# google/lasr

Hardware: AMD Instinct MI355X
Metric: rasterizer fwd+bwd frames/sec at 256x256, 2.3k faces (higher is better)
Workload: dtype f32

## Files before the change

lasr_amd/csrc/sr_backward.h:

```cpp
#pragma once
#include "sr_common.h"

namespace lasr {

constexpr bool BWD_FM = true;
#ifndef LASR_BWD_LDSREC
#define LASR_BWD_LDSREC 1
#endif
#ifndef LASR_BWD_WPE8
#define LASR_BWD_WPE8 0
#endif
#ifndef LASR_BWD_DIVREC
#define LASR_BWD_DIVREC 1
#endif
#ifndef LASR_BWD_ONE
#define LASR_BWD_ONE 1
#endif
constexpr int QCAP = 128;
constexpr int BWD_THREADS = 64;

template <bool LASR_FAST, int NCH>
__global__ __launch_bounds__(BWD_THREADS)
#if LASR_BWD_WPE8
__attribute__((amdgpu_waves_per_eu(LASR_FAST && NCH == 3 ? 8 : 1, LASR_FAST && NCH == 3 ? 8 : 8)))
#endif
void sr_backward_kernel(RasterArgs A, const float* __restrict__ colors,
                                                          const float* __restrict__ aggrs,
                                                          const float* __restrict__ gcolors,
                                                          float* __restrict__ gfaces, float* __restrict__ gtex)
{
    __shared__ unsigned int s_ring[BWD_THREADS / 64][QCAP];
#if LASR_BWD_LDSREC
    __shared__ __attribute__((aligned(16))) float s_rec[BWD_THREADS / 64][REC];
#endif
    constexpr bool FM = BWD_FM;
    const Modes m = LASR_FAST ? Modes{2, 1, 2, 1, 1} : A.m;
    if (A.near_far_dev) { A.near = A.near_far_dev[0]; A.far = A.near_far_dev[1]; }
    const int lane = threadIdx.x & 63;
    unsigned int* ring = s_ring[threadIdx.x >> 6];
#if defined(LASR_BWD_ORDER) && LASR_BWD_ORDER == 1
    int blk = xcd_remap(blockIdx.x, gridDim.x);
    {
        const int total = gridDim.x, per = total >> 3;
        if ((total & 7) == 0 && per % A.F == 0) {
            const int m = per / A.F, i = blockIdx.x >> 3, rank = i / m;
            blk = ((blockIdx.x & 7) * m + (i - rank * m)) * A.F + rank;
        }
    }
#elif defined(LASR_BWD_ORDER) && LASR_BWD_ORDER == 3
    const int blk = xcd_remap(blockIdx.x, gridDim.x);
#else
    int blk;
    {
        const int total = gridDim.x, per = total >> 3;
        blk = (total & 7) == 0 ? (blockIdx.x & 7) * per + (per - 1 - (blockIdx.x >> 3)) : total - 1 - blockIdx.x;
    }
#endif
    const int gw = __builtin_amdgcn_readfirstlane((int)((blk * blockDim.x + threadIdx.x) >> 6));
    if (gw >= A.N * A.F) return;
    const int bn = gw / A.F, fn = gw - bn * A.F;
    const int IS = A.IS, P = IS * IS;
    const cptr_t rec = as_const(A.recs + (size_t)gw * REC);
    const cptr_t tex = as_const(A.textures + (size_t)gw * A.T * NCH);
    const int flags = __float_as_int(rec[R_FLAGS]);
#if LASR_BWD_LDSREC
    typedef const float __attribute__((address_space(3)))* lptr_t;
    if (LASR_FAST && (flags & 16)) {
        float* dst = s_rec[threadIdx.x >> 6];
        if (lane < REC) dst[lane] = A.recs[(size_t)gw * REC + lane];
        __builtin_amdgcn_wave_barrier();
    }
    const lptr_t lrec = (lptr_t)s_rec[threadIdx.x >> 6];
#endif

    const unsigned rlo = (unsigned)__float_as_int(rec[R_BB + 0]), rext = (unsigned)__float_as_int(rec[R_BB + 1]);
    const int x0 = (int)(rlo & 0xffff), r0 = (int)(rlo >> 16);
    const int bw = (int)(rext & 0xffff) + 1, bh = (int)(rext >> 16) + 1;
    const bool empty = rlo == 0xffffffffu;
    const int npx = empty ? 0 : bw * bh;

    float gv[9] = {0, 0, 0, 0, 0, 0, 0, 0, 0};
    constexpr int NGT = 3 * NCH < 18 ? 18 : 3 * NCH;
    constexpr int THIRD = NCH == 9 ? 18 : 0;
    float gt[NGT];
#pragma unroll
    for (int k = 0; k < NGT; k++) gt[k] = 0.f;
    const bool front = (flags & 8) != 0;
    const bool vertex_tex = (m.tex == 1);
    const int lim = (A.N * A.F - gw) * A.T;
    const bool use_far = (m.dist == 2) && (flags & 16);
    const float thr_pad = A.thr * 1.05f;
    const float inv_is = A.inv_is;
    const bool pow2 = (IS & (IS - 1)) == 0;
    const float cx_a = A.cx_a, cx_b = A.cx_b, cy_b = A.cy_b;
    auto centre_x = [&](int xi) { return OPT_BWD_S1 && pow2 ? __builtin_fmaf((float)xi, cx_a, cx_b) : pix_center_p2(xi, IS, inv_is, pow2); };
    auto centre_y = [&](int row) { return OPT_BWD_S1 && pow2 ? __builtin_fmaf((float)row, -cx_a, cy_b) : pix_center_p2(IS - 1 - row, IS, inv_is, pow2); };
    float ld[9];
    const float far_t = A.far_t;
    if (OPT_BWD_S1 && use_far) {
#pragma unroll
        for (int k = 0; k < 3; k++) {
            const float h = __builtin_amdgcn_sqrtf(rec[R_HK2 + k]);
            ld[3 * k] = rec[R_INV + 3 * k] * h; ld[3 * k + 1] = rec[R_INV + 3 * k + 1] * h; ld[3 * k + 2] = rec[R_INV + 3 * k + 2] * h;
        }
    }
    const float tie_scale = (flags & 16) ? near_tie_scale(rec[R_HK2], rec[R_HK2 + 1], rec[R_HK2 + 2]) : 0.f;
    bool depth_safe = false;
    if (OPT_BWD_MATH && (flags & 16)) {
        const float z0 = rec[R_FACE + 2], z1 = rec[R_FACE + 5], z2 = rec[R_FACE + 8];
        const float zlo = fminf(fminf(z0, z1), z2), zhi = fmaxf(fmaxf(z0, z1), z2);
        depth_safe = zlo > 0.f && zlo * (1.f - 1e-4f) > A.near && zhi * (1.f + 1e-4f) < A.far;
    }
    auto ld_plane = [&](const float* base, int nplanes, int plane, int pn_) -> float {
#if defined(LASR_BWD_ABL) && LASR_BWD_ABL == 3
        return 0.25f + 1e-3f * (float)(pn_ & 255) + 0.01f * (float)plane;
#endif
        return base[((size_t)bn * nplanes + plane) * P + pn_];
    };

    int r = 0, c = 0;
#if LASR_BWD_DIVREC
    const int walk = __float_as_int(rec[15]);
    const int dr = empty ? 0 : walk >> 17, dc = empty ? 0 : 64 - dr * bw;
    if (!empty) { r = (lane * (walk & 0x1ffff)) >> 16; c = lane - r * bw; }
#else
    const int dr = empty ? 0 : 64 / bw, dc = empty ? 0 : 64 - dr * bw;
    if (!empty) { r = lane / bw; c = lane - r * bw; }
#endif

    int head = 0, tail = 0, base = 0;
    while (true) {
        if (base < npx) {
            const int xi = x0 + c, row = r0 + r;
            const bool in_range = base + lane < npx;
            c += dc; r += dr;
            if (c >= bw) { c -= bw; r += 1; }
            base += 64;
            bool keep = in_range;
            if (OPT_BWD_S1) {
                if (use_far) {
                    const float xp = __builtin_fmaf((float)xi, cx_a, cx_b), yp = __builtin_fmaf((float)row, -cx_a, cy_b);
                    const float d0 = __builtin_fmaf(ld[0], xp, __builtin_fmaf(ld[1], yp, ld[2]));
                    const float d1 = __builtin_fmaf(ld[3], xp, __builtin_fmaf(ld[4], yp, ld[5]));
                    const float d2 = __builtin_fmaf(ld[6], xp, __builtin_fmaf(ld[7], yp, ld[8]));
                    keep = in_range && !(fminf(fminf(d0, d1), d2) < far_t);
                }
            } else if (in_range && use_far) {
                float w0, w1, w2;
                barycentric(rec, pix_center_p2(xi, IS, inv_is, pow2), pix_center_p2(IS - 1 - row, IS, inv_is, pow2), w0, w1, w2);
                keep = !certainly_far(rec, w0, w1, w2, thr_pad);
            }
            const unsigned long long mask = wave_mask(keep);
            if (keep) ring[(tail + bits_below_lane(mask)) & (QCAP - 1)] = (unsigned)xi | ((unsigned)row << 16);
            tail += __popcll(mask);
        }
        const int avail = tail - head;
        if (!(avail >= 64 || (base >= npx && avail > 0))) {
            if (base >= npx) break;
            continue;
        }
        __builtin_amdgcn_wave_barrier();
        const bool active = lane < avail;
        const unsigned int packed = ring[(head + lane) & (QCAP - 1)];
        head += min(avail, 64);
#if defined(LASR_BWD_ABL) && LASR_BWD_ABL == 1
        gv[0] += (float)packed;
        continue;
#endif
        if (!active) continue;
        const int xi = packed & 0xffff, row = packed >> 16;
        const int pn = row * IS + xi;
        const float xp = centre_x(xi), yp = centre_y(row);

        float w0, w1, w2;
        Frag fr;
#if LASR_BWD_ONE
        if (LASR_FAST && (flags & 16)) {
#if LASR_BWD_LDSREC
            if (!fragment_one(lrec, A.thr, A.sigma, xp, yp, w0, w1, w2, fr, tie_scale)) continue;
#else
            if (!fragment_one(rec, A.thr, A.sigma, xp, yp, w0, w1, w2, fr, tie_scale)) continue;
#endif
        } else
#endif
        if (!fragment<FM, cptr_t, (OPT_BWD_MATH && LASR_FAST)>(rec, m.dist, A.thr, A.sigma, xp, yp, w0, w1, w2, fr)) continue;
        const float D = fr.D;
#if defined(LASR_BWD_ABL) && LASR_BWD_ABL == 2
        gv[0] += D + fr.dx + fr.dy + fr.t0 + fr.t1 + fr.t2 + fr.sign;
        continue;
#endif

        float Ca = ld_plane(gcolors, NCH + 1, NCH, pn);
        if (m.alpha == 1) Ca = div_<FM>(Ca, (float)A.F);
        else if (m.alpha == 2) {
            const float a_out = ld_plane(colors, NCH + 1, NCH, pn);
            Ca *= div_<FM>(1 - a_out, fmaxf(1 - D, 1e-6f));
        }
        float C = Ca;

        const float u0 = w0, u1 = w1, u2 = w2;
        if (vertex_tex) clip_normalise<FM, (OPT_BWD_MATH && LASR_FAST)>(w0, w1, w2); else clip_normalise<false>(w0, w1, w2);
        const float iz0r = rec[R_IZ + 0], iz1r = rec[R_IZ + 1], iz2r = rec[R_IZ + 2];
        const float q0 = w0 * iz0r, q1 = w1 * iz1r, q2 = w2 * iz2r;
        const float zp = OPT_BWD_MATH && LASR_FAST ? __builtin_amdgcn_rcpf(q0 + q1 + q2) : depth_at<FM>(rec, w0, w1, w2);
        if (!depth_safe) {
            float zc = zp;
            const float tol = 1e-4f * fabsf(zp);
            if (fabsf(zp - A.near) <= tol || fabsf(zp - A.far) <= tol) zc = depth_forward_exact(rec, xp, yp);
            if (zc < A.near || zc > A.far) continue;
        }

        float gz0 = 0, gz1 = 0, gz2 = 0;
        if (m.rgb == 0) {
            if ((float)fn == ld_plane(aggrs, 2, 1, pn)) {
                float g[NCH];
#pragma unroll
                for (int k = 0; k < NCH; k++) g[k] = ld_plane(gcolors, NCH + 1, k, pn);
                if (vertex_tex) {
#pragma unroll
                    for (int k = 0; k < NCH; k++) {
                        gt[k] += w0 * g[k]; gt[NCH + k] += w1 * g[k]; gt[2 * NCH + k] += w2 * g[k];
                    }
                } else {
                    const int j = surface_texel(w0, w1, A.res);
                    if (j >= 0 && j < A.T) {
                        float* gtp = gtex + (size_t)gw * A.T * 3 + 3 * j;
                        atomicAdd(gtp + 0, g[0]); atomicAdd(gtp + 1, g[1]); atomicAdd(gtp + 2, g[2]);
                    }
                }
            }
        } else if (front || m.double_side) {
            const float ssum = ld_plane(aggrs, 2, 0, pn);
            const float smax = ld_plane(aggrs, 2, 1, pn);
            const float zn = div_<FM>(A.far - zp, A.far - A.near);
            const float sm = div_<FM>(D * exp_<FM>(div_<FM>(zn - smax, A.gamma)), ssum);
            float g[NCH];
#pragma unroll
            for (int k = 0; k < NCH; k++) g[k] = ld_plane(gcolors, NCH + 1, k, pn);
            if (vertex_tex) {
#pragma unroll
                for (int k = 0; k < NCH; k++) {
                    gt[k] += sm * (w0 * g[k]); gt[NCH + k] += sm * (w1 * g[k]); gt[2 * NCH + k] += sm * (w2 * g[k]);
                }
            } else {
                const int j = surface_texel(w0, w1, A.res);
                if (j >= 0 && j < A.T) {
                    float* gtp = gtex + (size_t)gw * A.T * 3 + 3 * j;
                    atomicAdd(gtp + 0, sm * g[0]); atomicAdd(gtp + 1, sm * g[1]); atomicAdd(gtp + 2, sm * g[2]);
                }
            }
            float Crgb = 0.f;
#pragma unroll
            for (int k = 0; k < NCH; k++)
                Crgb += g[k] * (sample_colour(tex, w0, w1, w2, A.res, k, m.tex, lim, NCH) - ld_plane(colors, NCH + 1, k, pn));
            Crgb *= sm;
            C += div_<FM>(Crgb, D);
            const float Cz = div_<FM>(div_<FM>(Crgb, A.gamma), A.near - A.far) * zp * zp;
            if (OPT_BWD_MATH && LASR_FAST) {
                gz0 = Cz * q0 * iz0r; gz1 = Cz * q1 * iz1r; gz2 = Cz * q2 * iz2r;
            } else {
                const float iz0 = __builtin_amdgcn_rcpf(rec[R_FACE + 2]), iz1 = __builtin_amdgcn_rcpf(rec[R_FACE + 5]), iz2 = __builtin_amdgcn_rcpf(rec[R_FACE + 8]);
                gz0 = Cz * w0 * iz0 * iz0;
                gz1 = Cz * w1 * iz1 * iz1;
                gz2 = Cz * w2 * iz2 * iz2;
            }
        }

        C *= div_<FM>(D * (1 - D), A.sigma);
        float gx0 = 0, gy0 = 0, gx1 = 0, gy1 = 0, gx2 = 0, gy2 = 0;
        if (m.dist == 1) {
            const float t0 = fr.t0, t1 = fr.t1, t2 = fr.t2;
            const int p = t0 > t1 ? (t1 > t2 ? 2 : 1) : (t0 > t2 ? 2 : 0);
            const float ipx = rec[R_INV + 3 * p + 0], ipy = rec[R_INV + 3 * p + 1];
            const float dis = fr.dis;
            const float sc = 2.f * sqrtf(fabsf(dis));
            float gxy[3][2];
#pragma unroll
            for (int l = 0; l < 2; l++) {
                const float ipl = l == 0 ? ipx : ipy;
#pragma unroll
                for (int k = 0; k < 3; k++) {
                    float acc = 0.f;
                    acc += -ipl * rec[R_INV + 3 * k + 0] * xp;
                    acc += -ipl * rec[R_INV + 3 * k + 1] * yp;
                    acc += -ipl * rec[R_INV + 3 * k + 2] * 1.f;
                    gxy[k][l] = acc * C * sc;
                }
            }
            gx0 = gxy[0][0]; gy0 = gxy[0][1]; gx1 = gxy[1][0]; gy1 = gxy[1][1]; gx2 = gxy[2][0]; gy2 = gxy[2][1];
        } else if (m.dist == 2) {
            const float k2 = 2 * fr.sign * C;
            gx0 = k2 * (fr.t0 + u0) * fr.dx; gy0 = k2 * (fr.t0 + u0) * fr.dy;
            gx1 = k2 * (fr.t1 + u1) * fr.dx; gy1 = k2 * (fr.t1 + u1) * fr.dy;
            gx2 = k2 * (fr.t2 + u2) * fr.dx; gy2 = k2 * (fr.t2 + u2) * fr.dy;
        }
        gv[0] += gx0; gv[1] += gy0; gv[2] += gz0;
        gv[3] += gx1; gv[4] += gy1; gv[5] += gz1;
        gv[6] += gx2; gv[7] += gy2; gv[8] += gz2;
    }

    float v18[18], red[5];
    const int lane_row = lane >> 4;
    const int sub = lane_row == 0 ? 0 : lane_row == 1 ? 2 : lane_row == 2 ? 1 : 3;
    float* gf = gfaces + (size_t)gw * 9;
    float* gtp = gtex + (size_t)gw * 3 * NCH;
#pragma unroll
    for (int pass = 0; pass < (NCH > 3 ? 2 : 1); pass++) {
#pragma unroll
        for (int k = 0; k < 9; k++) {
            v18[k] = pass == 0 ? gv[k] : (vertex_tex ? gt[9 + k] : 0.f);
            v18[9 + k] = pass == 0 ? (vertex_tex ? gt[k] : 0.f) : (NCH == 9 && vertex_tex ? gt[THIRD + k] : 0.f);
        }
        wave_reduce18(v18, red);
        if ((lane & 15) == 15) {
#pragma unroll
            for (int i = 0; i < 5; i++) {
                if (i == 4 && (lane_row & 1)) continue;
                const int comp = i == 4 ? 16 + (lane_row >> 1) : 4 * i + sub;
                const bool ow = A.overwrite_grads && vertex_tex;
                if (pass == 0) {
                    if (comp < 9) gf[comp] = ow ? red[i] : gf[comp] + red[i];
                    else if (vertex_tex) gtp[comp - 9] = ow ? red[i] : gtp[comp - 9] + red[i];
                } else if ((comp < 9 || NCH == 9) && vertex_tex) gtp[9 + comp] = ow ? red[i] : gtp[9 + comp] + red[i];
            }
        }
    }
}

}
```

lasr_amd/csrc/sr_device.h:

```cpp
#pragma once
#include <hip/hip_runtime.h>

namespace lasr {

constexpr int REC = 48;

#ifndef LASR_OPT
#define LASR_OPT 0xffff
#endif
constexpr bool OPT_PKRECT = (LASR_OPT & 1) != 0;
constexpr bool OPT_MED3 = (LASR_OPT & 2) != 0;
constexpr bool OPT_NOSCALE = (LASR_OPT & 4) != 0;
constexpr bool OPT_SIGNFOLD = (LASR_OPT & 8) != 0;
constexpr bool OPT_SOFTMAX = (LASR_OPT & 16) != 0;
constexpr bool OPT_BWD_S1 = (LASR_OPT & 64) != 0;
constexpr bool OPT_BWD_MATH = (LASR_OPT & 128) != 0;
constexpr bool OPT_EDGESEL = (LASR_OPT & 256) != 0;
constexpr int R_BB = 0, R_FLAGS = 2, R_INV = 3, R_HK2 = 12, R_FACE = 16, R_DEN = 25, R_IDEN = 28, R_E = 32, R_IZ = 41;

typedef const float __attribute__((address_space(4)))* cptr_t;
__device__ __forceinline__ cptr_t as_const(const float* p) { return (cptr_t)(unsigned long long)p; }

struct Modes {
    int dist, rgb, alpha, tex, double_side;
// ... 189 lines not shown
    y = __builtin_fmaf(__builtin_fmaf(-b, y, 1.f), y, y);
#define LASR_QUOT(a)                                                     \
    {                                                                    \
        float q = a * y;                                                 \
        q = __builtin_fmaf(__builtin_fmaf(-b, q, a), y, q);              \
        a = __builtin_fmaf(__builtin_fmaf(-b, q, a), y, q);              \
    }
    LASR_QUOT(a0) LASR_QUOT(a1) LASR_QUOT(a2)
#undef LASR_QUOT
}

template <bool FM = false, bool TAME = false>
__device__ __forceinline__ void clip_normalise(float& w0, float& w1, float& w2)
{
    if (TAME) {
        w0 = __builtin_amdgcn_fmed3f(w0, 0.f, 1.f);
        w1 = __builtin_amdgcn_fmed3f(w1, 0.f, 1.f);
        w2 = __builtin_amdgcn_fmed3f(w2, 0.f, 1.f);
    } else {
        w0 = fmaxf(fminf(w0, 1.f), 0.f);
        w1 = fmaxf(fminf(w1, 1.f), 0.f);
        w2 = fmaxf(fminf(w2, 1.f), 0.f);
    }
    const float s = fmaxf(w0 + w1 + w2, 1e-5f);
    if (FM) { const float r = __builtin_amdgcn_rcpf(s); w0 *= r; w1 *= r; w2 *= r; }
    else div3_shared(w0, w1, w2, s);
}

template <bool FM> __device__ __forceinline__ float div_(float a, float b)
{
    return FM ? a * __builtin_amdgcn_rcpf(b) : a / b;
}
__device__ __forceinline__ float exp_1ulp(float x)
{
    const float L2E_HI = 1.44269502162933349609375f, L2E_LO = 1.925963033500011e-8f;
    const float n = rintf(x * L2E_HI);
    const float f = __builtin_fmaf(x, L2E_LO, __builtin_fmaf(x, L2E_HI, -n));
    return ldexpf(__builtin_amdgcn_exp2f(f), (int)n);
}
template <bool FM> __device__ __forceinline__ float exp_(float x) { return FM ? __expf(x) : exp_1ulp(x); }
template <bool FM, bool NOSCALE = false> __device__ __forceinline__ float sigmoid_neg_(float neg_arg)
{
    if (FM) return __builtin_amdgcn_rcpf(1.f + __expf(neg_arg));
    if (NOSCALE) return (float)recip64_noscale(1. + (double)exp_1ulp(neg_arg));
    return (float)(1. / (1. + (double)exp_1ulp(neg_arg)));
}

template <typename RP>
__device__ __forceinline__ bool certainly_far(RP rec, float w0, float w1, float w2, float thr_pad)
{
    return (w0 < 0.f && w0 * w0 * rec[R_HK2 + 0] > thr_pad) ||
           (w1 < 0.f && w1 * w1 * rec[R_HK2 + 1] > thr_pad) ||
           (w2 < 0.f && w2 * w2 * rec[R_HK2 + 2] > thr_pad);
}

template <int K, bool CLAMP, bool FM = false, bool MK = false, typename RP = cptr_t, bool IDEN = false>
__device__ __forceinline__ void edge_project(RP rec, float w0, float w1, float w2,
                                             float& u0, float& u1, float& u2)
{
#pragma clang fp contract(off)
    constexpr int B = (K + 1) % 3;
    const float e0 = rec[R_E + 3 * K + 0], e1 = rec[R_E + 3 * K + 1], e2 = rec[R_E + 3 * K + 2];
    const float eb = rec[R_E + 3 * K + B];
    const float num = w0 * e0 + w1 * e1 + w2 * e2 - eb;
    float ta = MK ? div_by_recip(num, rec[R_DEN + K], rec[R_IDEN + K])
                  : (FM && IDEN) ? num * rec[R_IDEN + K] : div_<FM>(num, rec[R_DEN + K]);
    float tb = 1 - ta;
    float tc = 0;
    if (CLAMP) {
        ta = fminf(fmaxf(ta, 0.f), 1.f);
        tb = fminf(fmaxf(tb, 0.f), 1.f);
    }
    float t[3];
    t[K] = ta; t[B] = tb; t[(K + 2) % 3] = tc;
    u0 = t[0] - w0; u1 = t[1] - w1; u2 = t[2] - w2;
}

struct Frag {
    float D;
    float sign, dx, dy;
    float t0, t1, t2;
    float dis;
    float narg;
};

template <bool FM = false, bool MK = false, typename RP = cptr_t, bool FWD = false, bool TAME = false, bool IDEN = false>
__device__ __forceinline__ bool euclid(RP rec, float xp, float yp,
                                       float w0, float w1, float w2, Frag& fr, float thr = 0.f)
{
#pragma clang fp contract(off)
    const float x0 = rec[R_FACE + 0], y0 = rec[R_FACE + 1], x1 = rec[R_FACE + 3], y1 = rec[R_FACE + 4], x2 = rec[R_FACE + 6], y2 = rec[R_FACE + 7];
    const bool inside = TAME ? (bool)((int)(fminf(fminf(w0, w1), w2) > 0) & (int)(fmaxf(fmaxf(w0, w1), w2) < 1))
                             : (w0 > 0 && w1 > 0 && w2 > 0 && w0 < 1 && w1 < 1 && w2 < 1);
    if (inside) {
        float best = 100000000.f, bx = 0, by = 0, b0 = 0, b1 = 0, b2 = 0;
        float u0, u1, u2;
#define LASR_TRY_EDGE(K)                                                          \
        edge_project<K, false, FM, MK, RP, IDEN>(rec, w0, w1, w2, u0, u1, u2);            \
        {                                                                         \
            const float px = u0 * x0 + u1 * x1 + u2 * x2;                         \
            const float py = u0 * y0 + u1 * y1 + u2 * y2;                         \
            const float d2 = px * px + py * py;                                   \
            if (d2 < best) { best = d2; bx = px; by = py; b0 = u0; b1 = u1; b2 = u2; } \
        }
        LASR_TRY_EDGE(0) LASR_TRY_EDGE(1) LASR_TRY_EDGE(2)
#undef LASR_TRY_EDGE
        if (FWD) { fr.narg = (-bx) * bx - by * by; return true; }
        fr.dx = bx; fr.dy = by; fr.t0 = b0; fr.t1 = b1; fr.t2 = b2; fr.sign = 1.f;
    } else {
        const int flags = __float_as_int(rec[R_FLAGS]);
        float u0, u1, u2;
        if (OPT_EDGESEL) {
            const bool n0 = w0 <= 0, n1 = w1 <= 0, n2 = w2 <= 0;
            bool o0 = false, o1 = false, o2 = false;
            if (flags & 7) {
                if (flags & 1) o0 = (xp - x0) * (x2 - x0) + (yp - y0) * (y2 - y0) > 0;
                if (flags & 2) o1 = (xp - x1) * (x0 - x1) + (yp - y1) * (y0 - y1) > 0;
                if (flags & 4) o2 = (xp - x2) * (x1 - x2) + (yp - y2) * (y1 - y2) > 0;
            }
            const bool c12 = n1 & n2, c20 = n2 & n0 & !n1, c01 = n0 & n1 & !n2;
            const bool e1 = (c20 & !o1) | (c01 & o2) | (n0 & !n1 & !n2);
            const bool e2 = (c01 & !o2) | (c12 & o0) | (n1 & !n0 & !n2);
            const bool e0 = !(e1 | e2);
            if (e0) edge_project<0, true, FM, MK, RP, IDEN>(rec, w0, w1, w2, u0, u1, u2);
            if (e1) edge_project<1, true, FM, MK, RP, IDEN>(rec, w0, w1, w2, u0, u1, u2);
            if (e2) edge_project<2, true, FM, MK, RP, IDEN>(rec, w0, w1, w2, u0, u1, u2);
        } else {
        int a = -1;
        if (w1 <= 0 && w2 <= 0) {
            a = 0;
            if ((flags & 1) && (xp - x0) * (x2 - x0) + (yp - y0) * (y2 - y0) > 0) a = 2;
        } else if (w2 <= 0 && w0 <= 0) {
            a = 1;
            if ((flags & 2) && (xp - x1) * (x0 - x1) + (yp - y1) * (y0 - y1) > 0) a = 0;
        } else if (w0 <= 0 && w1 <= 0) {
            a = 2;
            if ((flags & 4) && (xp - x2) * (x1 - x2) + (yp - y2) * (y1 - y2) > 0) a = 1;
        } else if (w0 <= 0) a = 1;
        else if (w1 <= 0) a = 2;
        else if (w2 <= 0) a = 0;
        if (a < 0) a = 0;
        if (a == 0) edge_project<0, true, FM, MK, RP, IDEN>(rec, w0, w1, w2, u0, u1, u2);
        else if (a == 1) edge_project<1, true, FM, MK, RP, IDEN>(rec, w0, w1, w2, u0, u1, u2);
        else edge_project<2, true, FM, MK, RP, IDEN>(rec, w0, w1, w2, u0, u1, u2);
        }
        fr.dx = u0 * x0 + u1 * x1 + u2 * x2;
        fr.dy = u0 * y0 + u1 * y1 + u2 * y2;
        if (FWD) { fr.narg = fr.dx * fr.dx + fr.dy * fr.dy; return !(fr.narg >= thr); }
        fr.t0 = u0; fr.t1 = u1; fr.t2 = u2; fr.sign = -1.f;
    }
    return true;
}

constexpr float NEAR_TIE = 0.985f;
constexpr float NEAR_TIE_ABS = 2.4e-6f;
__host__ __device__ __forceinline__ float near_tie_scale(float h2a, float h2b, float h2c)
{
    return 4.f * NEAR_TIE_ABS * NEAR_TIE_ABS / fminf(fminf(h2a, h2b), h2c);
}
__device__ __forceinline__ bool near_tie(float qlo, float qmid, float scale)
{
    const float gap = qmid - qlo;
    return (bool)((int)!(qlo < NEAR_TIE * qmid) | (int)!(gap * gap > scale * qmid));
}
#ifndef LASR_BWD_FMA
#define LASR_BWD_FMA 0
#endif
template <int K, typename RP>
__device__ __forceinline__ void edge_project_one(RP rec, float w0, float w1, float w2, float& u0, float& u1, float& u2)
{
#if !LASR_BWD_FMA
#pragma clang fp contract(off)
#endif
    constexpr int B = (K + 1) % 3;
    const float num = w0 * rec[R_E + 3 * K + 0] + w1 * rec[R_E + 3 * K + 1] + w2 * rec[R_E + 3 * K + 2] - rec[R_E + 3 * K + B];
    float ta = num * rec[R_IDEN + K];
    float tb = 1 - ta;
    ta = fminf(fmaxf(ta, 0.f), 1.f);
    tb = fminf(fmaxf(tb, 0.f), 1.f);
    float t[3];
    t[K] = ta; t[B] = tb; t[(K + 2) % 3] = 0;
    u0 = t[0] - w0; u1 = t[1] - w1; u2 = t[2] - w2;
}
template <typename RP>
__device__ __forceinline__ void euclid_one(RP rec, float xp, float yp, float w0, float w1, float w2, Frag& fr, float tie_scale)
{
#if !LASR_BWD_FMA
#pragma clang fp contract(off)
#endif
    const float x0 = rec[R_FACE + 0], y0 = rec[R_FACE + 1], x1 = rec[R_FACE + 3], y1 = rec[R_FACE + 4], x2 = rec[R_FACE + 6], y2 = rec[R_FACE + 7];
    const bool inside = (bool)((int)(fminf(fminf(w0, w1), w2) > 0) & (int)(fmaxf(fmaxf(w0, w1), w2) < 1));
    const int flags = __float_as_int(rec[R_FLAGS]);
    const bool n0 = w0 <= 0, n1 = w1 <= 0, n2 = w2 <= 0;
    bool o0 = false, o1 = false, o2 = false;
    if (flags & 7) {
        if (flags & 1) o0 = (xp - x0) * (x2 - x0) + (yp - y0) * (y2 - y0) > 0;
        if (flags & 2) o1 = (xp - x1) * (x0 - x1) + (yp - y1) * (y0 - y1) > 0;
        if (flags & 4) o2 = (xp - x2) * (x1 - x2) + (yp - y2) * (y1 - y2) > 0;
    }
    const bool c12 = n1 & n2, c20 = n2 & n0 & !n1, c01 = n0 & n1 & !n2;
    bool e1 = (c20 & !o1) | (c01 & o2) | (n0 & !n1 & !n2);
    bool e2 = (c01 & !o2) | (c12 & o0) | (n1 & !n0 & !n2);
    const float q0 = w2 * w2 * rec[R_HK2 + 2], q1 = w0 * w0 * rec[R_HK2 + 0], q2 = w1 * w1 * rec[R_HK2 + 1];
    const float qlo = fminf(fminf(q0, q1), q2), qmid = __builtin_amdgcn_fmed3f(q0, q1, q2);
    const bool tie = (bool)((int)inside & (int)near_tie(qlo, qmid, tie_scale));
    float u0, u1, u2;
    if (tie) {
        float best = 100000000.f, bx = 0, by = 0, b0 = 0, b1 = 0, b2 = 0;
#define LASR_TRY_EDGE(K)                                                          \
        edge_project<K, false, true, false, RP, true>(rec, w0, w1, w2, u0, u1, u2);   \
        {                                                                         \
            const float px = u0 * x0 + u1 * x1 + u2 * x2;                         \
            const float py = u0 * y0 + u1 * y1 + u2 * y2;                         \
            const float d2 = px * px + py * py;                                   \
            if (d2 < best) { best = d2; bx = px; by = py; b0 = u0; b1 = u1; b2 = u2; } \
        }
        LASR_TRY_EDGE(0) LASR_TRY_EDGE(1) LASR_TRY_EDGE(2)
#undef LASR_TRY_EDGE
        fr.dx = bx; fr.dy = by; u0 = b0; u1 = b1; u2 = b2;
    } else {
        const bool i1 = q1 == qlo, i2 = q2 == qlo;
        e1 = inside ? i1 : e1;
        e2 = inside ? i2 : e2;
        const bool e0 = !(e1 | e2);
        if (e0) edge_project_one<0>(rec, w0, w1, w2, u0, u1, u2);
        if (e1) edge_project_one<1>(rec, w0, w1, w2, u0, u1, u2);
        if (e2) edge_project_one<2>(rec, w0, w1, w2, u0, u1, u2);
        fr.dx = u0 * x0 + u1 * x1 + u2 * x2;
        fr.dy = u0 * y0 + u1 * y1 + u2 * y2;
    }
    fr.t0 = u0; fr.t1 = u1; fr.t2 = u2; fr.sign = inside ? 1.f : -1.f;
}

template <typename RP>
__device__ __forceinline__ void barycentric(RP rec, float xp, float yp, float& w0, float& w1, float& w2)
{
#pragma clang fp contract(off)
    w0 = rec[R_INV + 0] * xp + rec[R_INV + 1] * yp + rec[R_INV + 2];
    w1 = rec[R_INV + 3] * xp + rec[R_INV + 4] * yp + rec[R_INV + 5];
    w2 = rec[R_INV + 6] * xp + rec[R_INV + 7] * yp + rec[R_INV + 8];
}

template <bool FM = false, bool MK = false, typename RP = cptr_t, bool BT = false>
__device__ __forceinline__ bool fragment_w(RP rec, int dist, float thr, float sigma,
                                           float xp, float yp, float w0, float w1, float w2, Frag& fr,
                                           float inv_sigma = 0.f);

template <bool FM = false, typename RP = cptr_t, bool BT = false>
__device__ __forceinline__ bool fragment(RP rec, int dist, float thr, float sigma,
                                         float xp, float yp, float& w0, float& w1, float& w2, Frag& fr)
{
    barycentric(rec, xp, yp, w0, w1, w2);
    return fragment_w<FM, false, RP, BT>(rec, dist, thr, sigma, xp, yp, w0, w1, w2, fr);
}

template <bool FM, bool MK, typename RP, bool BT>
__device__ __forceinline__ bool fragment_w(RP rec, int dist, float thr, float sigma,
                                           float xp, float yp, float w0, float w1, float w2, Frag& fr, float inv_sigma)
{
#pragma clang fp contract(off)
    if (dist == 0) {
        if (!inside_closed(w0, w1, w2)) return false;
        fr.D = 1.f;
    } else if (dist == 1) {
        float d = w0 > w1 ? (w1 > w2 ? w2 : w1) : (w0 > w2 ? w2 : w0);
        d = d > 0 ? d * d : -(d * d);
        fr.dis = d; fr.t0 = w0; fr.t1 = w1; fr.t2 = w2;
        if (-d >= thr) return false;
        fr.D = sigmoid_neg_<FM>(MK ? div_by_recip(-d, sigma, inv_sigma) : div_<FM>(-d, sigma));
    } else if (!FM && MK && OPT_SIGNFOLD) {
        if (!euclid<FM, MK, RP, true, OPT_MED3>(rec, xp, yp, w0, w1, w2, fr, thr)) return false;
        fr.D = sigmoid_neg_<FM, OPT_NOSCALE>(div_by_recip(fr.narg, sigma, inv_sigma));
    } else {
        euclid<FM, MK, RP, false, (!FM && MK && OPT_MED3) || BT, BT>(rec, xp, yp, w0, w1, w2, fr);
        fr.dis = fr.dx * fr.dx + fr.dy * fr.dy;
        if (fr.sign < 0 && fr.dis >= thr) return false;
        fr.D = sigmoid_neg_<FM, (!FM && MK && OPT_NOSCALE)>(MK ? div_by_recip(-fr.sign * fr.dis, sigma, inv_sigma) : div_<FM>(-fr.sign * fr.dis, sigma));
    }
    return true;
}

template <typename RP>
__device__ __forceinline__ bool fragment_one(RP rec, float thr, float sigma, float xp, float yp, float& w0, float& w1, float& w2, Frag& fr,
                                             float tie_scale)
{
#if LASR_BWD_FMA
    w0 = rec[R_INV + 0] * xp + rec[R_INV + 1] * yp + rec[R_INV + 2];
    w1 = rec[R_INV + 3] * xp + rec[R_INV + 4] * yp + rec[R_INV + 5];
    w2 = rec[R_INV + 6] * xp + rec[R_INV + 7] * yp + rec[R_INV + 8];
#else
#pragma clang fp contract(off)
    barycentric(rec, xp, yp, w0, w1, w2);
#endif
    euclid_one(rec, xp, yp, w0, w1, w2, fr, tie_scale);
    fr.dis = fr.dx * fr.dx + fr.dy * fr.dy;
    if (fr.sign < 0 && fr.dis >= thr) return false;
    fr.D = sigmoid_neg_<true>(div_<true>(-fr.sign * fr.dis, sigma));
    return true;
}

template <bool FM = false, bool MK = false, typename RP = cptr_t>
__device__ __forceinline__ float depth_at(RP rec, float c0, float c1, float c2)
{
    if (MK) {
        const float s = div_by_recip(c0, rec[R_FACE + 2], rec[R_IZ + 0]) + div_by_recip(c1, rec[R_FACE + 5], rec[R_IZ + 1]) +
                        div_by_recip(c2, rec[R_FACE + 8], rec[R_IZ + 2]);
        return OPT_NOSCALE ? recip_noscale(s) : 1.f / s;
    }
    return div_<FM>(1.f, div_<FM>(c0, rec[R_FACE + 2]) + div_<FM>(c1, rec[R_FACE + 5]) + div_<FM>(c2, rec[R_FACE + 8]));
}

template <typename RP>
__device__ __forceinline__ float depth_forward_exact(RP rec, float xp, float yp)
{
#pragma clang fp contract(off)
    float w0 = rec[R_INV + 0] * xp + rec[R_INV + 1] * yp + rec[R_INV + 2];
    float w1 = rec[R_INV + 3] * xp + rec[R_INV + 4] * yp + rec[R_INV + 5];
    float w2 = rec[R_INV + 6] * xp + rec[R_INV + 7] * yp + rec[R_INV + 8];
    w0 = fmaxf(fminf(w0, 1.f), 0.f);
    w1 = fmaxf(fminf(w1, 1.f), 0.f);
    w2 = fmaxf(fminf(w2, 1.f), 0.f);
    const float s = fmaxf(w0 + w1 + w2, 1e-5f);
    w0 = w0 / s; w1 = w1 / s; w2 = w2 / s;
    return 1.f / (w0 / rec[R_FACE + 2] + w1 / rec[R_FACE + 5] + w2 / rec[R_FACE + 8]);
}

__device__ __forceinline__ int surface_texel(float c0, float c1, int res)
{
    const int ix = (int)(c0 * res), iy = (int)(c1 * res);
    if ((c0 + c1) * res - ix - iy <= 1) return iy * res + ix;
    return (res - 1 - iy) * res + (res - 1 - ix);
}

template <typename TP>
__device__ __forceinline__ float sample_colour(TP tex, float c0, float c1, float c2,
                                               int res, int ch, int tex_type, int lim, int nch = 3)
{
    if (tex_type == 0) {
        const int j = max(min(surface_texel(c0, c1, res), lim - 1), 0);
        return tex[j * 3 + ch];
    }
    return c0 * tex[ch] + c1 * tex[nch + ch] + c2 * tex[2 * nch + ch];
}

__device__ __forceinline__ unsigned long long wave_mask(bool c) { return __builtin_amdgcn_ballot_w64(c); }
__device__ __forceinline__ int bits_below_lane(unsigned long long m)
{
    return (int)__builtin_amdgcn_mbcnt_hi((unsigned)(m >> 32), __builtin_amdgcn_mbcnt_lo((unsigned)m, 0u));
}

__device__ __forceinline__ float wave_sum_to_lane63(float v)
{
#define LASR_DPP_ADD(ctrl, rmask, bmask)                                                              \
    v += __int_as_float(__builtin_amdgcn_update_dpp(0, __float_as_int(v), ctrl, rmask, bmask, false))
    LASR_DPP_ADD(0x111, 0xf, 0xf);
    LASR_DPP_ADD(0x112, 0xf, 0xf);
    LASR_DPP_ADD(0x114, 0xf, 0xe);
    LASR_DPP_ADD(0x118, 0xf, 0xc);
    LASR_DPP_ADD(0x142, 0xa, 0xf);
    LASR_DPP_ADD(0x143, 0xc, 0xf);
#undef LASR_DPP_ADD
    return v;
}

__device__ __forceinline__ float swap_add32(float a, float b)
{
    const auto r = __builtin_amdgcn_permlane32_swap(__float_as_uint(a), __float_as_uint(b), false, false);
    return __uint_as_float(r[0]) + __uint_as_float(r[1]);
}
__device__ __forceinline__ float swap_add16(float a, float b)
{
    const auto r = __builtin_amdgcn_permlane16_swap(__float_as_uint(a), __float_as_uint(b), false, false);
    return __uint_as_float(r[0]) + __uint_as_float(r[1]);
}
__device__ __forceinline__ float row_sum_to_lane15(float v)
{
#define LASR_DPP_ADD(ctrl, bmask) \
    v += __int_as_float(__builtin_amdgcn_update_dpp(0, __float_as_int(v), ctrl, 0xf, bmask, false))
    LASR_DPP_ADD(0x111, 0xf);
    LASR_DPP_ADD(0x112, 0xf);
    LASR_DPP_ADD(0x114, 0xe);
    LASR_DPP_ADD(0x118, 0xc);
#undef LASR_DPP_ADD
    return v;
}
__device__ __forceinline__ void wave_reduce18(const float (&v)[18], float (&out)[5])
{
    float s[9];
#pragma unroll
    for (int i = 0; i < 9; i++) s[i] = swap_add32(v[2 * i], v[2 * i + 1]);
#pragma unroll
    for (int i = 0; i < 4; i++) out[i] = row_sum_to_lane15(swap_add16(s[2 * i], s[2 * i + 1]));
    out[4] = row_sum_to_lane15(swap_add16(s[8], 0.f));
}

}
```

lasr_amd/csrc/sr_forward_pairs.h:

```cpp
#pragma once

namespace lasr {

constexpr int PW_CAP = 64;
constexpr int PW_LIST = 1024;
constexpr int PW_TILE = 16;

typedef unsigned long long u64_t;

constexpr int PR_INV = 0, PR_FLAGS = 9, PR_BB = 10, PR_ETBL = 11, PR_HK2 = 12, PR_BBE = 15, PR_XY = 16, PR_Z = 22, PR_IZ = 25, PR_OBT = 28, PR_EDGE = 32, PR_HQ = 56, PR_TEX = 60;

__host__ __device__ constexpr int pr_of(int i)
{
    return i == R_BB ? PR_BB : i == R_BB + 1 ? PR_BBE : i == R_FLAGS ? PR_FLAGS
         : (i >= R_INV && i < R_INV + 9) ? PR_INV + (i - R_INV)
         : (i >= R_HK2 && i < R_HK2 + 3) ? PR_HK2 + (i - R_HK2)
         : (i >= R_FACE && i < R_FACE + 9) ? ((i - R_FACE) % 3 == 2 ? PR_Z + (i - R_FACE) / 3 : PR_XY + 2 * ((i - R_FACE) / 3) + (i - R_FACE) % 3)
         : (i >= R_DEN && i < R_DEN + 3) ? PR_EDGE + 8 * (i - R_DEN) + 4
         : (i >= R_IDEN && i < R_IDEN + 3) ? PR_EDGE + 8 * (i - R_IDEN) + 5
         : (i >= R_E && i < R_E + 9) ? PR_EDGE + 8 * ((i - R_E) / 3) + (i - R_E) % 3
         : (i >= R_IZ && i < R_IZ + 3) ? PR_IZ + (i - R_IZ) : 15;
}
struct PairRecView {
    const float* p;
    __device__ __forceinline__ float operator[](int i) const { return p[pr_of(i)]; }
};

template <int NCH, int SPLIT = 1>
struct PairLds {
    static constexpr int Q0 = (PR_TEX + 3 * NCH + 3) / 4;
    static constexpr int RS = 4 * (Q0 | 1);
    float rec[SPLIT][PW_CAP * RS];
    unsigned short list[PW_LIST];
    int wcnt[2][4 * SPLIT];
    float sel[24];
    unsigned long long ball[SPLIT][2][16];
    float merge[SPLIT > 1 ? (SPLIT - 1) * 256 * (3 + NCH) : 1];
};

__device__ __forceinline__ float4 ld4(const float* p) { return *(const float4*)p; }
#ifndef LASR_PW_FENCE
#define LASR_PW_FENCE 0
#endif
#ifndef LASR_PW_WAVES
#define LASR_PW_WAVES 0
#endif
#define PW_LANDED(q) asm volatile("" : "+v"(q.x), "+v"(q.y), "+v"(q.z), "+v"(q.w))

template <typename RP>
__device__ __forceinline__ bool reaches_block(RP R, float xlo, float xhi, float ylo, float yhi, float thr_cull)
{
    bool hit = true;
    if (__float_as_int(R[R_FLAGS]) & 16) {
#pragma unroll
        for (int k = 0; k < 3; k++) {
            const float a = R[R_INV + 3 * k], b = R[R_INV + 3 * k + 1], c = R[R_INV + 3 * k + 2];
            const float w00 = a * xlo + b * ylo + c, w01 = a * xhi + b * ylo + c;
            const float w10 = a * xlo + b * yhi + c, w11 = a * xhi + b * yhi + c;
            const float wmax = fmaxf(fmaxf(w00, w01), fmaxf(w10, w11));
            if (wmax < 0.f && wmax * wmax * R[R_HK2 + k] > thr_cull) hit = false;
        }
    }
    return hit;
}

__host__ __device__ constexpr bool rec_used(int i) { return i < 15 || (i >= 16 && i < 31) || (i >= 32 && i < 44); }
template <int Q0, int Q1>
__device__ __forceinline__ void stage_quads(const float4* __restrict__ src, float* __restrict__ dst, float thr_far, bool well)
{
    float4 v[Q1 - Q0];
#pragma unroll
    for (int q = Q0; q < Q1; q++) v[q - Q0] = src[q];
#pragma unroll
    for (int q = Q0; q < Q1; q++) {
        const float w[4] = {v[q - Q0].x, v[q - Q0].y, v[q - Q0].z, v[q - Q0].w};
#pragma unroll
        for (int j = 0; j < 4; j++) {
            const int i = 4 * q + j;
            if (!rec_used(i)) continue;
            if (i >= R_HK2 && i < R_HK2 + 3) {
                dst[pr_of(i)] = well ? -sqrtf(thr_far / w[j]) : -__builtin_huge_valf();
                dst[PR_HQ + (i - R_HK2 + 1) % 3] = well ? w[j] : 0.f;
                if (i == R_HK2) dst[PR_HQ + 3] = near_tie_scale(w[0], w[1], w[2]);
                continue;
            }
            dst[pr_of(i)] = w[j];
            if (i == R_E + 1) dst[PR_EDGE + 3] = w[j];
            if (i == R_E + 5) dst[PR_EDGE + 8 + 3] = w[j];
            if (i == R_E + 6) dst[PR_EDGE + 16 + 3] = w[j];
        }
    }
}

__host__ __device__ constexpr unsigned edge_table(int obtuse_bits)
{
    unsigned t = 0;
    for (int over = 0; over < 2; over++)
        for (int idx = 0; idx < 8; idx++) {
            const bool n0 = idx & 1, n1 = idx & 2, n2 = idx & 4;
            const bool o0 = over && (obtuse_bits & 1), o1 = over && (obtuse_bits & 2), o2 = over && (obtuse_bits & 4);
            const bool c12 = n1 && n2, c20 = n2 && n0 && !n1, c01 = n0 && n1 && !n2;
            const bool e1 = (c20 && !o1) || (c01 && o2) || (n0 && !n1 && !n2);
            const bool e2 = (c01 && !o2) || (c12 && o0) || (n1 && !n0 && !n2);
            t |= (unsigned)((e1 ? 1 : 0) + (e2 ? 2 : 0)) << (2 * idx + 16 * over);
        }
    return t;
}

__device__ __forceinline__ float div_by_recip1(float a, float b, float y)
{
    const float q = a * y;
    return __builtin_fmaf(__builtin_fmaf(-b, q, a), y, q);
}

__device__ __forceinline__ float sigmoid_from_exp(float e)
{
    const double x = 1. + (double)e;
    const double y = __builtin_amdgcn_rcp(x);
    return (float)__builtin_fma(__builtin_fma(-x, y, 1.), y, y);
}

__device__ __forceinline__ float clamp01(float x)
{
    float r;
    asm("v_mul_f32_e64 %0, 1.0, %1 clamp" : "=v"(r) : "v"(x));
    return r;
}

template <int NCH>
__device__ __forceinline__ void merge_partial(PixState<NCH>& S, float pa, float pm, float ps, const float (&pc)[NCH],
                                              float gamma, float inv_gamma)
{
    S.a = (float)((double)S.a * (double)pa);
    const float mx = fmaxf(S.smax, pm);
    const float ds = S.smax - mx, dp = pm - mx;
    const float es = exp_1ulp(div_by_recip(ds, gamma, inv_gamma));
    const float ep = exp_1ulp(div_by_recip(dp, gamma, inv_gamma));
    S.ssum = S.ssum * es + ps * ep;
#pragma unroll
    for (int k = 0; k < NCH; k++) S.c[k] = S.c[k] * es + pc[k] * ep;
    S.smax = mx;
}

template <int NCH>
__device__ __forceinline__ void pair_apply(const RasterArgs& A, const UniRecip& U, const float* __restrict__ R, const float* __restrict__ SEL,
                                           bool is_in, bool has, float xp, float yp, PixState<NCH>& s)
{
#pragma clang fp contract(off)
    float4 q0 = ld4(R), q1 = ld4(R + 4), q2 = ld4(R + 8);
    float4 q4 = ld4(R + PR_XY), q5 = ld4(R + PR_XY + 4), ob = ld4(R + PR_OBT);
#if LASR_PW_FENCE & 1
    PW_LANDED(q0); PW_LANDED(q1); PW_LANDED(q2); PW_LANDED(q4); PW_LANDED(q5); PW_LANDED(ob);
#endif
    const float w0 = q0.x * xp + q0.y * yp + q0.z;
    const float w1 = q0.w * xp + q1.x * yp + q1.y;
    const float w2 = q1.z * xp + q1.w * yp + q2.x;
    const float x0 = q4.x, y0 = q4.y, x1 = q4.z, y1 = q4.w, x2 = q5.x, y2 = q5.y, z0 = q5.z, z1 = q5.w;
    float narg;
    bool tie = false;
    int k_in = 0;
    if (wave_mask(is_in) != 0) {
        const float4 hq = ld4(R + PR_HQ);
        const float g0 = w2 * w2 * hq.x, g1 = w0 * w0 * hq.y, g2 = w1 * w1 * hq.z;
        const float glo = fminf(fminf(g0, g1), g2), gmid = __builtin_amdgcn_fmed3f(g0, g1, g2);
        tie = (bool)((int)is_in & (int)near_tie(glo, gmid, hq.w));
        k_in = g1 == glo ? 1 : g2 == glo ? 2 : 0;
    }
    if (tie) {
        float best = 100000000.f, bx = 0, by = 0;
#pragma unroll
        for (int K = 0; K < 3; K++) {
            const float4 ea = ld4(R + PR_EDGE + 8 * K);
            const float2 eb = *(const float2*)(R + PR_EDGE + 8 * K + 4);
            const float num = w0 * ea.x + w1 * ea.y + w2 * ea.z - ea.w;
            const float ta = div_by_recip(num, eb.x, eb.y);
            const float tb = 1 - ta;
            float t[3];
            t[K] = ta; t[(K + 1) % 3] = tb; t[(K + 2) % 3] = 0;
            const float u0 = t[0] - w0, u1 = t[1] - w1, u2 = t[2] - w2;
            const float px = u0 * x0 + u1 * x1 + u2 * x2;
            const float py = u0 * y0 + u1 * y1 + u2 * y2;
            const float d2 = px * px + py * py;
            if (d2 < best) { best = d2; bx = px; by = py; }
        }
        narg = (-bx) * bx - by * by;
    } else {
        const bool over = (xp - ob.x) * ob.z + (yp - ob.y) * ob.w > 0;
        const int sh = (w0 <= 0 ? 2 : 0) | (w1 <= 0 ? 4 : 0) | (w2 <= 0 ? 8 : 0) | (over ? 16 : 0);
        int k = (int)__builtin_amdgcn_ubfe(__float_as_uint(q2.w), (unsigned)sh, 2u);
        k = is_in ? k_in : k;
        const float* E = R + PR_EDGE + 8 * k;
        const float4 ea = ld4(E);
        const float2 eb = *(const float2*)(E + 4);
        const float num = w0 * ea.x + w1 * ea.y + w2 * ea.z - ea.w;
        float ta = div_by_recip(num, eb.x, eb.y);
        float tb = 1 - ta;
        ta = clamp01(ta);
        tb = clamp01(tb);
        const float4 fa = ld4(SEL + 8 * k);
        const float2 fb = *(const float2*)(SEL + 8 * k + 4);
        const float t0 = __builtin_fmaf(tb, fa.w, ta * fa.x), t1 = __builtin_fmaf(tb, fb.x, ta * fa.y), t2 = __builtin_fmaf(tb, fb.y, ta * fa.z);
        const float u0 = t0 - w0, u1 = t1 - w1, u2 = t2 - w2;
        const float dx = u0 * x0 + u1 * x1 + u2 * x2;
        const float dy = u0 * y0 + u1 * y1 + u2 * y2;
        const float d2 = dx * dx + dy * dy;
        narg = is_in ? -d2 : d2;
        if ((bool)((int)!is_in & ((int)(d2 >= A.thr) | (int)!has))) return;
    }
    float4 q6 = ld4(R + PR_XY + 8);
    float4 tq[(3 * NCH + 3) / 4];
#pragma unroll
    for (int q = 0; q < (3 * NCH + 3) / 4; q++) tq[q] = ld4(R + PR_TEX + 4 * q);
    const float D = sigmoid_from_exp(exp_1ulp(div_by_recip1(narg, A.sigma, U.inv_sigma)));
    s.a = __builtin_fmaf(-s.a, D, s.a);
#if LASR_PW_FENCE & 2
    PW_LANDED(q6);
#pragma unroll
    for (int q = 0; q < (3 * NCH + 3) / 4; q++) PW_LANDED(tq[q]);
#endif
    float c0 = clamp01(w0), c1 = clamp01(w1), c2 = clamp01(w2);
    {
        const float sm = fmaxf(c0 + c1 + c2, 1e-5f);
        float y = __builtin_amdgcn_rcpf(sm);
        y = __builtin_fmaf(__builtin_fmaf(-sm, y, 1.f), y, y);
        c0 = div_by_recip1(c0, sm, y); c1 = div_by_recip1(c1, sm, y); c2 = div_by_recip1(c2, sm, y);
    }
    const float zs = div_by_recip1(c0, z0, q6.y) + div_by_recip1(c1, z1, q6.z) + div_by_recip1(c2, q6.x, q6.w);
    float zp;
    {
        float y = __builtin_amdgcn_rcpf(zs);
        y = __builtin_fmaf(__builtin_fmaf(-zs, y, 1.f), y, y);
        zp = __builtin_fmaf(__builtin_fmaf(-zs, y, 1.f), y, y);
    }
    if (!(zp >= A.near && zp <= A.far)) return;
    const float zn = div_by_recip1(A.far - zp, A.far - A.near, U.inv_fmn);
    const bool up = zn > s.smax;
    const float d = -fabsf(zn - s.smax);
    const float Ex = exp_1ulp(div_by_recip1(d, A.gamma, U.inv_gamma));
    const float hist = up ? Ex : 1.f, wgt = up ? D : Ex * D;
    s.smax = max_finite(zn, s.smax);
    s.ssum = __builtin_fmaf(hist, s.ssum, wgt);
    float tex[3 * NCH];
#pragma unroll
    for (int q = 0; q < (3 * NCH + 3) / 4; q++) {
        const float4 t = tq[q];
        tex[4 * q] = t.x;
        if (4 * q + 1 < 3 * NCH) tex[4 * q + 1] = t.y;
        if (4 * q + 2 < 3 * NCH) tex[4 * q + 2] = t.z;
        if (4 * q + 3 < 3 * NCH) tex[4 * q + 3] = t.w;
    }
#pragma unroll
    for (int k = 0; k < NCH; k++) {
        const float col = __builtin_fmaf(c2, tex[2 * NCH + k], __builtin_fmaf(c1, tex[NCH + k], c0 * tex[k]));
        s.c[k] = __builtin_fmaf(wgt, col, hist * s.c[k]);
    }
}

__device__ __forceinline__ int rank_of(int k)
{
    u64_t Gm = ~0ull;
// ... 409 lines not shown
```

Baseline: 102,700.

## Use edge lookup table and single precomputed projection in backward fragment

```diff
diff --git a/lasr_amd/csrc/sr_backward.h b/lasr_amd/csrc/sr_backward.h
--- a/lasr_amd/csrc/sr_backward.h
+++ b/lasr_amd/csrc/sr_backward.h
@@ -31,7 +31,7 @@
 {
     __shared__ unsigned int s_ring[BWD_THREADS / 64][QCAP];
 #if LASR_BWD_LDSREC
-    __shared__ __attribute__((aligned(16))) float s_rec[BWD_THREADS / 64][REC];
+    __shared__ __attribute__((aligned(16))) float s_rec[BWD_THREADS / 64][REC + (LASR_FAST ? BX : 0)];
 #endif
     constexpr bool FM = BWD_FM;
     const Modes m = LASR_FAST ? Modes{2, 1, 2, 1, 1} : A.m;
@@ -68,6 +68,9 @@
     if (LASR_FAST && (flags & 16)) {
         float* dst = s_rec[threadIdx.x >> 6];
         if (lane < REC) dst[lane] = A.recs[(size_t)gw * REC + lane];
+#if LASR_BWD_ONE && (LASR_BWD_TBL || LASR_BWD_ONEPROJ)
+        dst[REC + lane] = bwd_ext_word(A.recs + (size_t)gw * REC, flags, lane);
+#endif
         __builtin_amdgcn_wave_barrier();
     }
     const lptr_t lrec = (lptr_t)s_rec[threadIdx.x >> 6];
@@ -177,7 +180,11 @@
 #if LASR_BWD_ONE
         if (LASR_FAST && (flags & 16)) {
 #if LASR_BWD_LDSREC
+#if LASR_BWD_TBL || LASR_BWD_ONEPROJ
+            if (!fragment_one_ext(lrec, lrec + REC, flags, A.thr, A.sigma, xp, yp, w0, w1, w2, fr, tie_scale)) continue;
+#else
             if (!fragment_one(lrec, A.thr, A.sigma, xp, yp, w0, w1, w2, fr, tie_scale)) continue;
+#endif
 #else
             if (!fragment_one(rec, A.thr, A.sigma, xp, yp, w0, w1, w2, fr, tie_scale)) continue;
 #endif
diff --git a/lasr_amd/csrc/sr_device.h b/lasr_amd/csrc/sr_device.h
--- a/lasr_amd/csrc/sr_device.h
+++ b/lasr_amd/csrc/sr_device.h
@@ -365,6 +365,53 @@
     return true;
 }
 
+__host__ __device__ constexpr unsigned edge_table(int obtuse_bits)
+{
+    unsigned t = 0;
+    for (int over = 0; over < 2; over++)
+        for (int idx = 0; idx < 8; idx++) {
+            const bool n0 = idx & 1, n1 = idx & 2, n2 = idx & 4;
+            const bool o0 = over && (obtuse_bits & 1), o1 = over && (obtuse_bits & 2), o2 = over && (obtuse_bits & 4);
+            const bool c12 = n1 && n2, c20 = n2 && n0 && !n1, c01 = n0 && n1 && !n2;
+            const bool e1 = (c20 && !o1) || (c01 && o2) || (n0 && !n1 && !n2);
+            const bool e2 = (c01 && !o2) || (c12 && o0) || (n1 && !n0 && !n2);
+            t |= (unsigned)((e1 ? 1 : 0) + (e2 ? 2 : 0)) << (2 * idx + 16 * over);
+        }
+    return t;
+}
+
+__host__ __device__ constexpr bool edge_table_matches()
+{
+    for (int v = 0; v < 4; v++) {
+        const int ob = v == 0 ? 0 : 1 << (v - 1);
+        const unsigned tbl = edge_table(ob);
+        for (int over = 0; over < 2; over++)
+            for (int idx = 0; idx < 8; idx++) {
+                const int k = (int)((tbl >> (2 * idx + 16 * over)) & 3u);
+                const bool n0 = idx & 1, n1 = idx & 2, n2 = idx & 4;
+                const bool o0 = over && (ob & 1), o1 = over && (ob & 2), o2 = over && (ob & 4);
+                const bool c12 = n1 & n2, c20 = n2 & n0 & !n1, c01 = n0 & n1 & !n2;
+                const bool e1 = (c20 & !o1) | (c01 & o2) | (n0 & !n1 & !n2);
+                const bool e2 = (c01 & !o2) | (c12 & o0) | (n1 & !n0 & !n2);
+                const bool e0 = !(e1 | e2);
+                if ((int)e0 + (int)e1 + (int)e2 != 1) return false;
+                if (k != (e1 ? 1 : e2 ? 2 : 0)) return false;
+                int a = -1;
+                if (n1 && n2) { a = 0; if (o0) a = 2; }
+                else if (n2 && n0) { a = 1; if (o1) a = 0; }
+                else if (n0 && n1) { a = 2; if (o2) a = 1; }
+                else if (n0) a = 1;
+                else if (n1) a = 2;
+                else if (n2) a = 0;
+                if (a < 0) a = 0;
+                if (k != a) return false;
+                if (idx == 0 && k != 0) return false;
+            }
+    }
+    return true;
+}
+static_assert(edge_table_matches(), "edge_table disagrees with euclid_one's edge choice");
+
 constexpr float NEAR_TIE = 0.985f;
 constexpr float NEAR_TIE_ABS = 2.4e-6f;
 __host__ __device__ __forceinline__ float near_tie_scale(float h2a, float h2b, float h2c)
@@ -439,6 +486,115 @@
         if (e0) edge_project_one<0>(rec, w0, w1, w2, u0, u1, u2);
         if (e1) edge_project_one<1>(rec, w0, w1, w2, u0, u1, u2);
         if (e2) edge_project_one<2>(rec, w0, w1, w2, u0, u1, u2);
+        fr.dx = u0 * x0 + u1 * x1 + u2 * x2;
+        fr.dy = u0 * y0 + u1 * y1 + u2 * y2;
+    }
+    fr.t0 = u0; fr.t1 = u1; fr.t2 = u2; fr.sign = inside ? 1.f : -1.f;
+}
+
+#ifndef LASR_BWD_TBL
+#define LASR_BWD_TBL 1
+#endif
+#ifndef LASR_BWD_ONEPROJ
+#define LASR_BWD_ONEPROJ 1
+#endif
+#ifndef LASR_BWD_TSEL
+#define LASR_BWD_TSEL 0
+#endif
+constexpr int BX = 64, BX_STRIDE = 16, BX_OBT = 12;
+typedef float f4_t __attribute__((ext_vector_type(4)));
+typedef const float __attribute__((address_space(3)))* lds_cptr_t;
+typedef const f4_t __attribute__((address_space(3)))* lds_c4ptr_t;
+__device__ __forceinline__ float bwd_ext_word(const float* __restrict__ f, int flags, int L)
+{
+    const int k = L >> 4, i = L & 15;
+    const int c = (flags & 1) ? 0 : (flags & 2) ? 1 : 2, o = c == 0 ? 2 : c - 1;
+    const bool obt = L >= BX_OBT && L < BX_OBT + 4;
+    int ia = i < 3 ? R_E + 3 * k + i : i == 3 ? (k == 2 ? R_E + 6 : R_E + 4 * k + 1) : R_IDEN + k;
+    ia = obt ? R_FACE + 3 * ((L & 2) ? o : c) + (L & 1) : ia;
+    const int ib = R_FACE + 3 * c + (L & 1);
+    const float a = f[ia], b = f[ib];
+    float v = (obt && (L & 2)) ? a - b : a;
+    const int kb = k == 2 ? 0 : k + 1;
+    if (i >= 5 && i < 8) v = (i - 5 == k) ? 1.f : 0.f;
+    if (i >= 8 && i < 11) v = (i - 8 == kb) ? 1.f : 0.f;
+    return v;
+}
+__host__ __device__ constexpr unsigned edge_table_of_flags(int flags)
+{
+    return (flags & 1) ? edge_table(1) : (flags & 2) ? edge_table(2) : (flags & 4) ? edge_table(4) : edge_table(0);
+}
+__device__ __forceinline__ void euclid_one_ext(lds_cptr_t rec, lds_cptr_t ext, int flags, float xp, float yp, float w0, float w1, float w2,
+                                               Frag& fr, float tie_scale)
+{
+#if !LASR_BWD_FMA
+#pragma clang fp contract(off)
+#endif
+    const float x0 = rec[R_FACE + 0], y0 = rec[R_FACE + 1], x1 = rec[R_FACE + 3], y1 = rec[R_FACE + 4], x2 = rec[R_FACE + 6], y2 = rec[R_FACE + 7];
+    const bool inside = (bool)((int)(fminf(fminf(w0, w1), w2) > 0) & (int)(fmaxf(fmaxf(w0, w1), w2) < 1));
+    const float q0 = w2 * w2 * rec[R_HK2 + 2], q1 = w0 * w0 * rec[R_HK2 + 0], q2 = w1 * w1 * rec[R_HK2 + 1];
+    const float qlo = fminf(fminf(q0, q1), q2), qmid = __builtin_amdgcn_fmed3f(q0, q1, q2);
+    const bool tie = (bool)((int)inside & (int)near_tie(qlo, qmid, tie_scale));
+    float u0, u1, u2;
+    if (tie) {
+        float best = 100000000.f, bx = 0, by = 0, b0 = 0, b1 = 0, b2 = 0;
+#define LASR_TRY_EDGE(K)                                                          \
+        edge_project<K, false, true, false, lds_cptr_t, true>(rec, w0, w1, w2, u0, u1, u2);   \
+        {                                                                         \
+            const float px = u0 * x0 + u1 * x1 + u2 * x2;                         \
+            const float py = u0 * y0 + u1 * y1 + u2 * y2;                         \
+            const float d2 = px * px + py * py;                                   \
+            if (d2 < best) { best = d2; bx = px; by = py; b0 = u0; b1 = u1; b2 = u2; } \
+        }
+        LASR_TRY_EDGE(0) LASR_TRY_EDGE(1) LASR_TRY_EDGE(2)
+#undef LASR_TRY_EDGE
+        fr.dx = bx; fr.dy = by; u0 = b0; u1 = b1; u2 = b2;
+    } else {
+#if LASR_BWD_TBL
+        const bool i1 = (bool)((int)inside & (int)(q1 == qlo)), i2 = (bool)((int)inside & (int)(q2 == qlo));
+        bool over = false;
+        if (flags & 7) {
+            const f4_t ob = *(lds_c4ptr_t)(ext + BX_OBT);
+            over = (xp - ob.x) * ob.z + (yp - ob.y) * ob.w > 0;
+        }
+        const int sh = (w0 <= 0 ? 2 : 0) | (w1 <= 0 ? 4 : 0) | (w2 <= 0 ? 8 : 0) | (over ? 16 : 0);
+        const int k = (int)__builtin_amdgcn_ubfe(edge_table_of_flags(flags), (unsigned)sh, 2u) | (i1 ? 1 : 0) | (i2 ? 2 : 0);
+#else
+        const bool i1 = q1 == qlo, i2 = q2 == qlo;
+        const bool n0 = w0 <= 0, n1 = w1 <= 0, n2 = w2 <= 0;
+        bool o0 = false, o1 = false, o2 = false;
+        if (flags & 7) {
+            if (flags & 1) o0 = (xp - x0) * (x2 - x0) + (yp - y0) * (y2 - y0) > 0;
+            if (flags & 2) o1 = (xp - x1) * (x0 - x1) + (yp - y1) * (y0 - y1) > 0;
+            if (flags & 4) o2 = (xp - x2) * (x1 - x2) + (yp - y2) * (y1 - y2) > 0;
+        }
+        const bool c12 = n1 & n2, c20 = n2 & n0 & !n1, c01 = n0 & n1 & !n2;
+        bool e1 = (c20 & !o1) | (c01 & o2) | (n0 & !n1 & !n2);
+        bool e2 = (c01 & !o2) | (c12 & o0) | (n1 & !n0 & !n2);
+        e1 = inside ? i1 : e1;
+        e2 = inside ? i2 : e2;
+        const int k = e2 ? 2 : e1 ? 1 : 0;
+#endif
+#if LASR_BWD_ONEPROJ
+        const lds_cptr_t E = ext + BX_STRIDE * k;
+        const f4_t ea = *(lds_c4ptr_t)E;
+        const float num = w0 * ea.x + w1 * ea.y + w2 * ea.z - ea.w;
+        float ta = num * E[4];
+        float tb = 1 - ta;
+        ta = fminf(fmaxf(ta, 0.f), 1.f);
+        tb = fminf(fmaxf(tb, 0.f), 1.f);
+#if LASR_BWD_TSEL
+        const float t0 = k == 0 ? ta : k == 2 ? tb : 0.f, t1 = k == 1 ? ta : k == 0 ? tb : 0.f, t2 = k == 2 ? ta : k == 1 ? tb : 0.f;
+#else
+        const f4_t fa = *(lds_c4ptr_t)(E + 4), fb = *(lds_c4ptr_t)(E + 8);
+        const float t0 = __builtin_fmaf(tb, fb.x, ta * fa.y), t1 = __builtin_fmaf(tb, fb.y, ta * fa.z), t2 = __builtin_fmaf(tb, fb.z, ta * fa.w);
+#endif
+        u0 = t0 - w0; u1 = t1 - w1; u2 = t2 - w2;
+#else
+        if (k == 0) edge_project_one<0>(rec, w0, w1, w2, u0, u1, u2);
+        if (k == 1) edge_project_one<1>(rec, w0, w1, w2, u0, u1, u2);
+        if (k == 2) edge_project_one<2>(rec, w0, w1, w2, u0, u1, u2);
+#endif
         fr.dx = u0 * x0 + u1 * x1 + u2 * x2;
         fr.dy = u0 * y0 + u1 * y1 + u2 * y2;
     }
@@ -512,6 +668,24 @@
     return true;
 }
 
+__device__ __forceinline__ bool fragment_one_ext(lds_cptr_t rec, lds_cptr_t ext, int flags, float thr, float sigma, float xp, float yp,
+                                                 float& w0, float& w1, float& w2, Frag& fr, float tie_scale)
+{
+#if LASR_BWD_FMA
+    w0 = rec[R_INV + 0] * xp + rec[R_INV + 1] * yp + rec[R_INV + 2];
+    w1 = rec[R_INV + 3] * xp + rec[R_INV + 4] * yp + rec[R_INV + 5];
+    w2 = rec[R_INV + 6] * xp + rec[R_INV + 7] * yp + rec[R_INV + 8];
+#else
+#pragma clang fp contract(off)
+    barycentric(rec, xp, yp, w0, w1, w2);
+#endif
+    euclid_one_ext(rec, ext, flags, xp, yp, w0, w1, w2, fr, tie_scale);
+    fr.dis = fr.dx * fr.dx + fr.dy * fr.dy;
+    if (fr.sign < 0 && fr.dis >= thr) return false;
+    fr.D = sigmoid_neg_<true>(div_<true>(-fr.sign * fr.dis, sigma));
+    return true;
+}
+
 template <bool FM = false, bool MK = false, typename RP = cptr_t>
 __device__ __forceinline__ float depth_at(RP rec, float c0, float c1, float c2)
 {
diff --git a/lasr_amd/csrc/sr_forward_pairs.h b/lasr_amd/csrc/sr_forward_pairs.h
--- a/lasr_amd/csrc/sr_forward_pairs.h
+++ b/lasr_amd/csrc/sr_forward_pairs.h
@@ -92,20 +92,6 @@
     }
 }
 
-__host__ __device__ constexpr unsigned edge_table(int obtuse_bits)
-{
-    unsigned t = 0;
-    for (int over = 0; over < 2; over++)
-        for (int idx = 0; idx < 8; idx++) {
-            const bool n0 = idx & 1, n1 = idx & 2, n2 = idx & 4;
-            const bool o0 = over && (obtuse_bits & 1), o1 = over && (obtuse_bits & 2), o2 = over && (obtuse_bits & 4);
-            const bool c12 = n1 && n2, c20 = n2 && n0 && !n1, c01 = n0 && n1 && !n2;
-            const bool e1 = (c20 && !o1) || (c01 && o2) || (n0 && !n1 && !n2);
-            const bool e2 = (c01 && !o2) || (c12 && o0) || (n1 && !n0 && !n2);
-            t |= (unsigned)((e1 ? 1 : 0) + (e2 ? 2 : 0)) << (2 * idx + 16 * over);
-        }
-    return t;
-}
 
 __device__ __forceinline__ float div_by_recip1(float a, float b, float y)
 {
```

Result: faster. 103,900, median of 6 (+1.2%).
